# candrewlee14/zgml

Hardware: AMD Instinct MI355X
Metric: decode_tokens_per_sec (higher is better)
Workload: dtype f32; 1 GPU; SmolLM-135M Q4_0 greedy decode, batch 1, 1xMI355X (BASELINE configs[1]); weights=synthetic Q4_0 (int4 + f16 block scale / 32), tied f32 LM head, max_seq=2048, loop=device-resident (inputs in HBM), parallelism=none

## Files before the change

include/zgml_hip.h:

```cpp
#ifndef ZGML_HIP_H
#define ZGML_HIP_H

#include <stddef.h>
#include <stdint.h>

#ifdef __cplusplus
extern "C" {
#endif

#define ZGML_HIP_ABI_VERSION 1

enum {
    ZGML_OP_NONE = 0,
    ZGML_OP_VIEW = 1,
    ZGML_OP_RESHAPE = 2,
    ZGML_OP_TRANSPOSE = 3,
    ZGML_OP_PERMUTE = 4,
    ZGML_OP_AS_STRIDED = 5,
    ZGML_OP_BROADCAST_TO = 6,
    ZGML_OP_ADD = 7,
    ZGML_OP_MUL = 8,
    ZGML_OP_NEG = 9,
    ZGML_OP_ABS = 10,
    ZGML_OP_SGN = 11,
// ... 261 lines not shown


uint64_t zgml_hip_program_plan_text(zgml_hip_ctx* ctx, zgml_hip_program* handle, char* out, uint64_t cap);

enum {
    ZGML_HIP_OPT_FUSION = 1,
    ZGML_HIP_OPT_GRAPH = 2,
    ZGML_HIP_OPT_PROFILE = 3,
    ZGML_HIP_OPT_SKIP_DEAD_UPLOADS = 4,
    ZGML_HIP_OPT_F16_DENSE_WEIGHTS = 5,
    ZGML_HIP_OPT_DENSE_WEIGHT_CACHE = 6,
    ZGML_HIP_OPT_ATTN_SPLIT_MIN_KEYS = 7,
    ZGML_HIP_OPT_FUSE_RESIDENT_WGS = 8,
    ZGML_HIP_OPT_KSPLIT = 9,
    ZGML_HIP_OPT_W8A8 = 10,
    ZGML_HIP_OPT_SMALL_M_MATVEC = 11
};
int zgml_hip_set_option(zgml_hip_ctx* ctx, int option, int64_t value);
void zgml_hip_dense_cache_invalidate(zgml_hip_ctx* ctx, const float* b);
void zgml_hip_dense_cache_stats(zgml_hip_ctx* ctx, uint64_t* hits, uint64_t* misses, uint64_t* bytes);

void* zgml_hip_program_buffer_ptr(zgml_hip_program* handle, uint16_t buf_idx);
int zgml_hip_copy_program_buffer(zgml_hip_ctx* ctx, zgml_hip_program* dst, uint16_t dst_buf, uint64_t dst_offset,
                                 zgml_hip_program* src, uint16_t src_buf, uint64_t src_offset, uint64_t n_elems);
void* zgml_hip_stream(zgml_hip_ctx* ctx);
void zgml_hip_enqueue_program(zgml_hip_ctx* ctx, zgml_hip_program* handle);
void zgml_hip_enqueue_ops(zgml_hip_ctx* ctx, zgml_hip_program* handle, uint64_t first, uint64_t count);
int zgml_hip_program_set_barriers(zgml_hip_ctx* ctx, zgml_hip_program* handle, const uint64_t* op_indices,
                                  uint64_t n);
void zgml_hip_synchronize(zgml_hip_ctx* ctx);
int zgml_hip_stage_inputs(zgml_hip_ctx* ctx, zgml_hip_program* handle, const zgml_program_io* inputs, uint64_t n_inputs);
// ... 122 lines not shown
```

zgml_amd/capi.py:

```python
from __future__ import annotations

import ctypes as C
import os
from pathlib import Path

ABI_VERSION = 1

OP = {
    "none": 0, "view": 1, "reshape": 2, "transpose": 3, "permute": 4, "as_strided": 5,
    "broadcast_to": 6, "add": 7, "mul": 8, "neg": 9, "abs": 10, "sgn": 11, "step": 12,
    "relu": 13, "sqrt": 14, "recip": 15, "exp": 16, "log": 17, "gelu": 18, "sum": 19,
    "max": 20, "repeat": 21,
}
OP_NAME = {v: k for k, v in OP.items()}

DOP_KINDS = [
    "elementwise", "matmul", "qmatmul", "softmax", "layernorm", "rmsnorm", "reduce",
    "repeat", "slice_assign", "rope", "attention", "fused_elementwise",
]
DOP = {name: i for i, name in enumerate(DOP_KINDS)}
DOP.update({"kvq_store": 13, "attention_kvq": 14})


class MatMulGeom(C.Structure):
# ... 187 lines not shown
class ShardPointC(C.Structure):
    _fields_ = [("op_end", C.c_uint64), ("buf_idx", C.c_uint16), ("_pad", C.c_uint16), ("offset", C.c_uint32),
                ("len_per_rank", C.c_uint32)]


class ShardPeerHandleC(C.Structure):
    _fields_ = [("ipc", C.c_ubyte * 64), ("pid", C.c_uint64), ("raw", C.c_uint64), ("bytes", C.c_uint64)]


OPT_FUSION, OPT_GRAPH, OPT_PROFILE, OPT_SKIP_DEAD_UPLOADS, OPT_F16_DENSE_WEIGHTS, OPT_DENSE_WEIGHT_CACHE = 1, 2, 3, 4, 5, 6
OPT_ATTN_SPLIT_MIN_KEYS = 7
OPT_FUSE_RESIDENT_WGS = 8
OPT_KSPLIT = 9
OPT_W8A8 = 10
OPT_SMALL_M_MATVEC = 11

_PKG_DIR = Path(__file__).resolve().parent
HIP_LIB_PATH = _PKG_DIR / "lib" / "libzgml_hip.so"
HOST_LIB_PATH = Path(os.environ["ZGML_HOST_LIB"]) if os.environ.get("ZGML_HOST_LIB") else _PKG_DIR / "lib" / "libzgml_host.so"

_hip_lib = None


def _bind_hip(lib: C.CDLL) -> None:
    vp, u64, u32, i32 = C.c_void_p, C.c_uint64, C.c_uint32, C.c_int
    lib.zgml_hip_create.restype, lib.zgml_hip_create.argtypes = vp, [i32]
    lib.zgml_hip_destroy.restype, lib.zgml_hip_destroy.argtypes = None, [vp]
    lib.zgml_hip_last_error.restype, lib.zgml_hip_last_error.argtypes = C.c_char_p, [vp]
    lib.zgml_hip_clear_error.restype, lib.zgml_hip_clear_error.argtypes = None, [vp]
    lib.zgml_hip_capabilities.restype, lib.zgml_hip_capabilities.argtypes = None, [C.POINTER(CapabilitiesC)]
# ... 120 lines not shown
```

zgml_amd/csrc/kernels.h:

```cpp
#pragma once

#include <hip/hip_runtime.h>
#include <stdint.h>
#include <stdlib.h>

#include "../../include/zgml_hip.h"
#include "switches.h"

namespace zgml {

inline uint32_t device_cus() {
    static const uint32_t n = [] {
        int dev = 0, cus = 0;
        if (hipGetDevice(&dev) != hipSuccess || hipDeviceGetAttribute(&cus, hipDeviceAttributeMultiprocessorCount, dev) != hipSuccess || cus <= 0) cus = 256;
        return (uint32_t)cus;
    }();
    return n;
}

constexpr int kMaxFusedSteps = 8;

struct FusedStepDev {
    uint32_t op;
    uint32_t swapped;
// ... 402 lines not shown
uint32_t qmatmul_max_group();
void launch_qmatmul_group(hipStream_t s, const QWeightDev* w, const QMatmulParams* p, uint32_t n, float* scratch);
bool qmv_prenorm_ok(const QWeightDev& w, uint32_t K, uint64_t total_cols, uint32_t M);
bool qmv_pair_ok(const QWeightDev& w);
bool qmv_can_group(const QWeightDev& a, const QWeightDev& b);
uint32_t qmv_max_prologue_k(const QWeightDev& w);
void launch_qmatvec_fused(hipStream_t s, const QmvLaunch& L);
bool launch_qkv_attention(hipStream_t s, const QmvLaunch& L, const AttnDecodeParams* dev_params, uint32_t n_heads, uint32_t n_kv, uint32_t d_head,
                          const AttnSplit& sp, uint32_t* counters, const uint32_t* idx, uint32_t* seen, uint32_t* timeout,
                          const QmvLaunch* o_proj = nullptr, uint32_t* out_cnt = nullptr, uint32_t* o_seen = nullptr, bool kvq = false);
bool launch_attention_o(hipStream_t s, const AttnDecodeParams* dev_params, uint32_t n_heads, uint32_t d_head, const AttnSplit& sp, const QmvLaunch& o_proj,
                        uint32_t* out_cnt, uint32_t* o_seen, uint32_t* timeout);
int attn_o_blocks_per_cu(uint32_t d_head);
int qkv_attn_kon_census(hipStream_t s, uint32_t d_head, bool kvq, uint32_t grid);
int qkv_attn_kon_blocks_per_cu(uint32_t d_head, bool kvq);
void launch_synth_packed(hipStream_t s, const QWeightDev& w, uint32_t matrix_id);

struct KsVec {
    const float* base = nullptr;
    const float* parts = nullptr;
    uint32_t n_parts = 0;
    float* sum_dst = nullptr;
    float* add_dst = nullptr;
};
struct KsNormIn {
    KsVec x;
    const float* gamma = nullptr;
    float eps = 0.f;
    float* store_mid = nullptr;
    float* store_x = nullptr;
// ... 69 lines not shown
```

zgml_amd/csrc/plan.hip:

```cpp
#include "runtime_internal.h"

namespace {

float* buf_at(zgml_hip_program* p, uint16_t idx, uint64_t off) { return p->bufs[idx] + off; }

template <typename T>
const T* upload_params(zgml_hip_program* p, const std::vector<T>& v) {
    void* d = nullptr;
    if (hipMalloc(&d, v.size() * sizeof(T)) != hipSuccess) {
        p->ctx->fail("plan: parameter array allocation failed");
        return nullptr;
    }
    if (h2d_sync(p->ctx->stream, d, v.data(), v.size() * sizeof(T)) != hipSuccess) p->ctx->fail("plan: parameter array upload failed");
    p->param_blobs.push_back(d);
    return (const T*)d;
}

AttnSplit attn_split_for(zgml_hip_program* p, uint32_t n_heads, uint32_t d_head, uint32_t max_kv, int default_min_keys = 128) {
    const int want = sw().hip_attn_split;
    const int min_keys_env = sw().hip_attn_split_min_keys;
    AttnSplit sp;
    const int64_t min_keys = p->ctx->opt_attn_split_min_keys >= 0 ? p->ctx->opt_attn_split_min_keys : (min_keys_env >= 0 ? min_keys_env : default_min_keys);
    if (min_keys == 0 || want <= 1) return sp;
    sp.min_keys = (uint32_t)std::min<int64_t>(std::max<int64_t>(32, min_keys), 1 << 30);
// ... 899 lines not shown
        bool ok = ga.n_epi == 5 && st[0].op == ZGML_OP_NEG && !st[0].store && st[1].op == ZGML_OP_EXP && st[1].store && st[2].op == ZGML_OP_ADD &&
                  st[2].operand && st[2].operand != ga.dst && st[2].operand != st[1].store && !st[2].store && st[3].op == ZGML_OP_RECIP && !st[3].store &&
                  st[4].op == ZGML_OP_MUL && st[4].operand == ga.dst && st[4].store && up.n_epi == 0;
        ok = ok && ga.w.format == up.w.format && qmv_pair_ok(ga.w) && qmv_pair_ok(up.w) && ga.w.N == up.w.N && ga.w.K == up.w.K && (ga.w.N / 16) % 2 == 0 && ga.w.N == D->K &&
             (G->pro.kind == QMV_PRO_NONE || G->pro.kind == QMV_PRO_PRENORM) && D->n_parts == 1;
        ok = ok && ((D->pro.a == st[4].store && D->pro.b == up.dst) || (D->pro.b == st[4].store && D->pro.a == up.dst));
        ok = ok && (ga.w.format == QW_Q4K || G->pro.kind != QMV_PRO_PRENORM || ga.w.N >= G->K);
        ok = ok && (const char*)up.w.qs == (const char*)ga.w.qs + ga.w.qs_bytes && (const char*)up.w.sc == (const char*)ga.w.sc + ga.w.sc_bytes;
        ok = ok && ((uintptr_t)G->pro.a % 16 == 0) && (G->K % 4 == 0) && (G->pro.kind != QMV_PRO_PRENORM || (uintptr_t)G->pro.xg % 16 == 0);
        if (!ok) continue;
        if (barrier_between_launches(p, i - 1)) continue;
        G->pair_out = D->pro.store_x;
        QmvPrologue plain;
        plain.a = D->pro.store_x;
        D->pro = plain;
    }
}

struct Planner {
    zgml_hip_program* p;
    const std::vector<zgml_device_op>& ops;
    const std::vector<OpAccess>& access;
    const size_t n;
    std::vector<int> owner;
    std::vector<char> in_macro;
    std::vector<Macro> macros;
    struct ProInfo {
        QmvPrologue pro;
        std::vector<uint32_t> absorbed;
        std::vector<uint32_t> consumers;
// ... 772 lines not shown
void build_fused_plan(zgml_hip_program* p) {
    Planner pl(p);
    pl.hoist_constant_repeats();
    pl.prologues();
    pl.matvec_macros();
    pl.decode_attention(false);
    pl.decode_attention(true);
    pl.store_folds();
    pl.row_chains();
    pl.elementwise_chains();
    pl.singletons();
    pl.emit_levels();
    fuse_ksplit(p);
    arm_prenorm(p);
    arm_pair(p);
    fuse_qkv_attention(p);
#ifdef ZGML_TRACE
    fuse_attention_o(p);
#endif
}

}

namespace zgml_rt {

void free_param_blobs(zgml_hip_program* p) {
    for (void* d : p->param_blobs) hipFree(d);
    p->param_blobs.clear();
}

void build_plan(zgml_hip_program* p) {
    {
        hipStreamCaptureStatus st = hipStreamCaptureStatusNone;
        if (hipStreamIsCapturing(p->ctx->stream, &st) == hipSuccess && st != hipStreamCaptureStatusNone) {
            p->ctx->fail("build_plan: the plan has to be rebuilt, but the context's stream is being captured — run one step outside the capture first");
            return;
        }
    }
    hipStreamSynchronize(p->ctx->stream);
    p->plan.clear();
    for (size_t i = 0; i < p->ops.size(); i++) {
        const zgml_device_op& op = p->ops[i];
        if (op.kind == ZGML_DOP_QMATMUL && op.u.qmatmul.M != 1 && op.u.qmatmul.M > p->kon_max_m && op.u.qmatmul.weight_idx < p->qweights.size() &&
            p->qweights[op.u.qmatmul.weight_idx].format == QW_Q4K)
            p->ctx->fail("build_plan: op " + std::to_string(i) + " is an M > " + std::to_string(p->kon_max_m) + " qmatmul over a weight packed for M <= " +
                         std::to_string(p->kon_max_m) + " mat-vecs (K-on-lanes layout)");
    }
    free_param_blobs(p);
    for (void* d : p->fuse_owned) hipFree(d);
    p->fuse_owned.clear();
    p->fuse_epoch = p->ctx->fuse_epoch;
    p->split_buf = nullptr, p->split_cnt = nullptr, p->split_buf_floats = 0, p->split_cnt_words = 0;
    p->split_pos = UINT64_MAX - 1, p->split_input = nullptr, p->qmm_group = nullptr, p->f16_group = nullptr;
    p->plan_batched = p->ctx->opt_fusion && p->batching_safe;
    if (p->plan_batched) {
// ... 23 lines not shown
```

zgml_amd/csrc/qmatvec.hip:

```cpp
#include "qmv_common.h"
#include "attention_decode.h"

#include <hip/hip_fp16.h>
#include <math.h>
#include <stdlib.h>
#include <string.h>

#include <type_traits>
#include <utility>

namespace zgml {

namespace {



struct QMVPartDev {
    const uint4* qs;
    const void* sc;
    float* out;
    uint32_t NB2;
    uint32_t block_begin;
    uint32_t out_rs;
    uint32_t n_epi;
// ... 1496 lines not shown
                         : (fused_kvq ? qkv_attn_kernel<__half, true, 16, true> : qkv_attn_kernel<__half, true, 16, false>);
        else
            ff = prenorm ? (fused_kvq ? qkv_attn_kernel<__half, true, 32, true, 2> : qkv_attn_kernel<__half, true, 32, false, 2>)
                         : (fused_kvq ? qkv_attn_kernel<__half, true, 32, true> : qkv_attn_kernel<__half, true, 32, false>);
        hipLaunchKernelGGL(ff, dim3(total_blocks + extra_blocks), dim3(1024), lds, s, a.parts[0].qs, a.parts[0].sc, a.parts[0].out, head_xa, head_xb, a.in_rs, a.K,
                           head_flags(a, waves, true, rmsnorm, late), nb2_12, a, f);
        return true;
    }
    hipLaunchKernelGGL(fn, grid, dim3(waves * 64), lds, s, a.parts[0].qs, a.parts[0].sc, a.parts[0].out, head_xa, head_xb, a.in_rs, a.K,
                       head_flags(a, waves, contig, rmsnorm, late), nb2_12, a);
    return true;
}

}

uint32_t qmv_max_prologue_k(const QWeightDev& w) { return w.format == QW_Q4K ? UINT32_MAX : kMaxWaves * 64 * 4 * kXRegs; }

void launch_qmatvec_rows(hipStream_t s, const QWeightDev& w, const QMatmulParams& p, bool xvec) {
    QMVArgs a{};
    a.n_parts = 1;
    a.parts[0].qs = (const uint4*)w.qs;
    a.parts[0].sc = w.sc;
    a.parts[0].out = p.dst;
    a.parts[0].NB2 = p.N / 16;
    a.parts[0].block_begin = 0;
    a.parts[0].out_rs = p.dst_rs;
    a.parts[0].n_epi = 0;
    a.pro.kind = QMV_PRO_NONE;
    a.pro.a = p.input;
    a.pro.b = p.input;
// ... 168 lines not shown
```

zgml_amd/csrc/runtime.hip:

```cpp
#include "runtime_internal.h"

namespace zgml_rt {
std::string g_create_error;
}

namespace {


void fill_caps(zgml_capabilities* c) {
    memset(c, 0, sizeof(*c));
    c->compiled_programs = 1;
    c->host_visible_program_memory = 0;
    c->dense_matmul_f32 = 1;
    c->dense_matmul_f16 = 1;
    c->qmatmul = 1;
    c->fused_elementwise = 1;
    c->max_fused_elementwise_steps_has = 1;
    c->max_fused_elementwise_steps = kMaxFusedSteps;
    c->f16_weight_promotion = 1;
    c->dynamic_program_refresh = 1;
    c->prefill_attention = 1;
    c->decode_attention = 1;
    c->quantized_kv = 1;
    c->command_buffer_execution = 1;
// ... 573 lines not shown

int zgml_hip_set_option(zgml_hip_ctx* ctx, int option, int64_t value) {
    if (!ctx) return -1;
    switch (option) {
        case ZGML_HIP_OPT_FUSION: ctx->opt_fusion = value != 0; return 0;
        case ZGML_HIP_OPT_GRAPH: ctx->opt_graph = value != 0; return 0;
        case ZGML_HIP_OPT_PROFILE: ctx->opt_profile = value != 0; return 0;
        case ZGML_HIP_OPT_SKIP_DEAD_UPLOADS: ctx->opt_skip_dead = value != 0; return 0;
        case ZGML_HIP_OPT_F16_DENSE_WEIGHTS: ctx->opt_f16_dense = value != 0; return 0;
        case ZGML_HIP_OPT_ATTN_SPLIT_MIN_KEYS: ctx->opt_attn_split_min_keys = value < 0 ? -1 : value; return 0;
        case ZGML_HIP_OPT_FUSE_RESIDENT_WGS:
            ctx->opt_fuse_resident_wgs = value < 0 ? -1 : value;
            ctx->fuse_epoch++;
            return 0;
        case ZGML_HIP_OPT_KSPLIT: ctx->opt_ksplit = value != 0; return 0;
        case ZGML_HIP_OPT_W8A8: ctx->opt_w8a8 = value != 0; return 0;
        case ZGML_HIP_OPT_SMALL_M_MATVEC:
            ctx->opt_small_m = value <= 0 ? 0 : (value == 1 ? kKonRowsRoutedM : (uint32_t)std::min<int64_t>(value, kKonRowsMaxM));
            return 0;
        case ZGML_HIP_OPT_DENSE_WEIGHT_CACHE:
            ctx->b_cache_cap = value > 0 ? (uint64_t)value : 0;
            if (!ctx->b_cache_cap) ctx->drop_b_cache();
            return 0;
        default: return -1;
    }
}

int zgml_hip_dense_matmul_f32(zgml_hip_ctx* ctx, float* dst, uint64_t dst_len, const float* a, uint64_t a_len,
                              const float* b, uint64_t b_len, const zgml_matmul_geom* g) {
    if (!ctx || !g || !dst || !a || !b) return 0;
// ... 73 lines not shown
    if (hits) *hits = ctx->b_cache_hits;
    if (misses) *misses = ctx->b_cache_misses;
    if (bytes) *bytes = ctx->b_cache_bytes;
}

zgml_hip_program* zgml_hip_compile_program(zgml_hip_ctx* ctx, const zgml_device_program* prog) {
    if (!ctx || !prog) return nullptr;
    if (!program_supported(prog)) {
        ctx->fail("compile_program: program not supported by Capabilities.hip");
        return nullptr;
    }
    hipSetDevice(ctx->device);
    zgml_hip_program* p = new zgml_hip_program();
    p->ctx = ctx;
    p->ksplit = ctx->opt_ksplit;
    own_ops(p, prog->ops, prog->n_ops);
    const size_t nb = prog->n_buffers;
    p->sizes.resize(nb);
    for (size_t i = 0; i < nb; i++) p->sizes[i] = prog->buffer_sizes[i] ? prog->buffer_sizes[i] : 1;

    std::vector<char> live(nb, ctx->opt_skip_dead ? 0 : 1);
    std::vector<uint16_t> ids;
    std::vector<char> qw_live(prog->n_qweights, 0);
    for (const auto& op : p->ops) {
        ids.clear();
        op_buffers(op, ids);
        for (uint16_t id : ids) live[id] = 1;
        if (op.kind == ZGML_DOP_QMATMUL) qw_live[op.u.qmatmul.weight_idx] = 1;
    }

// ... 713 lines not shown
        ctx->fail("copy_program_buffer: range exceeds a buffer");
        return -1;
    }
    unhoist_if_guarded(dst, dst_buf);
    hipSetDevice(ctx->device);
    return CTX_CHECK(ctx, hipMemcpyAsync(dst->bufs[dst_buf] + dst_offset, src->bufs[src_buf] + src_offset, n_elems * sizeof(float),
                                         hipMemcpyDeviceToDevice, ctx->stream))
               ? 0
               : -1;
}

void zgml_hip_enqueue_ops(zgml_hip_ctx* ctx, zgml_hip_program* p, uint64_t first, uint64_t count) {
    if (!ctx || !p) return;
    hipSetDevice(ctx->device);
    if (!p->ksplit_off && !(first == 0 && count >= p->ops.size()))
        p->ksplit_off = true, p->plan_dirty = p->plan_dirty || p->has_deferred;
    ensure_plan(p);
    flush_dyn(p);
    for (auto& L : p->plan) {
        if (L.op_lo >= first && L.op_hi < first + count) {
            L.run(ctx->stream);
        } else if (!(L.op_hi < first || L.op_lo >= first + count)) {
            ctx->fail("enqueue_ops: range cuts through a batched launch; declare it with zgml_hip_program_set_barriers");
            return;
        }
    }
}

int zgml_hip_program_set_barriers(zgml_hip_ctx* ctx, zgml_hip_program* p, const uint64_t* op_indices, uint64_t n) {
    if (!ctx || !p) return -1;
    p->barriers.assign(op_indices, op_indices + n);
// ... 21 lines not shown
```

zgml_amd/csrc/runtime_internal.h:

```cpp
#pragma once
#include <hip/hip_runtime.h>

#include <algorithm>
#include <chrono>
#include <cstdio>
#include <cstdlib>
#include <cstring>
#include <functional>
#include <map>
#include <memory>
#include <string>
#include <vector>

#include "kernels.h"
#include "schedule.h"

using namespace zgml;

namespace zgml_rt {

extern std::string g_create_error;

struct SplitHook {
    const float* out = nullptr;
// ... 47 lines not shown
    bool dyn_row = false;
};

}
using namespace zgml_rt;

struct ShardState;
struct zgml_hip_ctx {
    int device = 0;
    hipStream_t stream = nullptr;
    std::string err;
    bool opt_fusion = true, opt_graph = true, opt_profile = false, opt_skip_dead = true, opt_f16_dense = false;
    bool host_prof = false;
    uint64_t prof_ns[4] = {0, 0, 0, 0}, prof_calls[4] = {0, 0, 0, 0};
    bool opt_ksplit = false;
    bool opt_w8a8 = false;
    uint32_t opt_small_m = 0;
    int64_t opt_attn_split_min_keys = -1;
    int64_t opt_fuse_resident_wgs = -1;
    float *mm_a = nullptr, *mm_b = nullptr, *mm_c = nullptr;
    uint64_t mm_a_cap = 0, mm_b_cap = 0, mm_c_cap = 0;
    struct CachedB {
        float* dev;
        uint64_t span;
    };
    std::map<const float*, CachedB> b_cache;
    uint64_t b_cache_cap = 0, b_cache_bytes = 0, b_cache_hits = 0, b_cache_misses = 0;
    void drop_b_cache() {
        for (auto& kv : b_cache) hipFree(kv.second.dev);
        b_cache.clear();
        b_cache_bytes = 0;
    }
    float* arg_val = nullptr;
    int64_t* arg_idx = nullptr;
    uint32_t* arg_cnt = nullptr;
    int64_t* arg_out = nullptr;
    int64_t* arg_out_host = nullptr;
    uint64_t* smp_keys = nullptr;
    SampleParamsDev* smp_params = nullptr;
    uint32_t* smp_out = nullptr;
    struct ShardState* shard = nullptr;
    uint32_t* handoff_flag = nullptr;
    uint32_t* handoff_flag_dev = nullptr;
    bool fuse_qkv_off = false;
    uint64_t fuse_epoch = 0;
    int n_cu = 0;
    std::map<uint64_t, int> census;
    bool handoff_ok(const char* where) {
        if (!handoff_flag || !*(volatile uint32_t*)handoff_flag) return true;
        const uint32_t cause = *(volatile uint32_t*)handoff_flag;
        *(volatile uint32_t*)handoff_flag = 0;
        if (cause == 2) {
            fail(std::string(where) + ": a peer gather's wait at a gather point timed out (or a peer had already failed the step) — the results of "
                                      "this step are wrong on every rank; all ranks must re-attach (zgml_hip_shard_attach + peer export / import) before stepping again");
            return false;
        }
        fuse_qkv_off = true, fuse_epoch++;
        fail(std::string(where) + ": an in-launch hand-off wait of a fused q/k/v + attention launch timed out — the results of this run are wrong; "
                                  "the fusion is now off for this context (later runs use two launches)");
        return false;
    }

    void fail(const std::string& what) {
        if (err.empty()) err = what;
    }
    bool check(hipError_t e, const char* what) {
        if (e == hipSuccess) return true;
        fail(std::string(what) + ": " + hipGetErrorString(e));
        return false;
// ... 27 lines not shown
    uint64_t split_buf_floats = 0, split_cnt_words = 0;
    bool f16_stream_nt = false;
    std::vector<void*> f16_weights;
    std::vector<void*> owned;
    uint64_t fuse_epoch = 0;
    std::vector<void*> fuse_owned;
    std::vector<char> hoist_op;
    std::vector<char> hoist_guard;
    bool hoist_ok = true;
    bool ksplit = false;
    uint32_t kon_max_m = 1;
    uint32_t n_seqs = 0;
    std::vector<uint32_t> op_seq;
    bool ksplit_off = false;
    bool has_deferred = false;
    float* prenorm_buf = nullptr;
    size_t prenorm_bytes = 0;
    float* scratch = nullptr;
    uint64_t scratch_bytes = 0;
    uint64_t split_pos = UINT64_MAX - 1;
    const float* split_input = nullptr;
    std::shared_ptr<std::vector<std::pair<QWeightDev, QMatmulParams>>> qmm_group;
    std::shared_ptr<std::vector<DenseF16Params>> f16_group;
    uint32_t split_M = 0, split_K = 0, split_in_rs = 0, split_kind = 0;
    uint32_t* dyn_dev = nullptr;
    uint32_t* dyn_host = nullptr;
    bool dyn_dirty = true;
    std::vector<Launch> plan;
    bool plan_dirty = true;
    Schedule sched;
// ... 69 lines not shown
```

Measured before the change: 1672 tokens/s.

## Fuse post-attention O, gate/up and down matvecs into one XCD-local chained launch

```diff
diff --git a/include/zgml_hip.h b/include/zgml_hip.h
--- a/include/zgml_hip.h
+++ b/include/zgml_hip.h
@@ -299,7 +299,8 @@
     ZGML_HIP_OPT_FUSE_RESIDENT_WGS = 8,
     ZGML_HIP_OPT_KSPLIT = 9,
     ZGML_HIP_OPT_W8A8 = 10,
-    ZGML_HIP_OPT_SMALL_M_MATVEC = 11
+    ZGML_HIP_OPT_SMALL_M_MATVEC = 11,
+    ZGML_HIP_OPT_XCD_CHAIN = 12
 };
 int zgml_hip_set_option(zgml_hip_ctx* ctx, int option, int64_t value);
 void zgml_hip_dense_cache_invalidate(zgml_hip_ctx* ctx, const float* b);
diff --git a/zgml_amd/capi.py b/zgml_amd/capi.py
--- a/zgml_amd/capi.py
+++ b/zgml_amd/capi.py
@@ -225,6 +225,7 @@
 OPT_KSPLIT = 9
 OPT_W8A8 = 10
 OPT_SMALL_M_MATVEC = 11
+OPT_XCD_CHAIN = 12
 
 _PKG_DIR = Path(__file__).resolve().parent
 HIP_LIB_PATH = _PKG_DIR / "lib" / "libzgml_hip.so"
diff --git a/zgml_amd/csrc/kernels.h b/zgml_amd/csrc/kernels.h
--- a/zgml_amd/csrc/kernels.h
+++ b/zgml_amd/csrc/kernels.h
@@ -440,6 +440,20 @@
 int attn_o_blocks_per_cu(uint32_t d_head);
 int qkv_attn_kon_census(hipStream_t s, uint32_t d_head, bool kvq, uint32_t grid);
 int qkv_attn_kon_blocks_per_cu(uint32_t d_head, bool kvq);
+uint32_t qmv_waves_of(const QWeightDev& w);
+
+constexpr bool kXcdChainDefault = true;
+struct XcdChainLaunch {
+    QmvLaunch o, gu, down;
+    uint32_t* sync = nullptr;
+    uint32_t* timeout = nullptr;
+    uint32_t P = 32, target_xcc = 0, grid = 256;
+    unsigned long long* trace = nullptr;
+};
+bool xcd_chain_shape_ok(const QmvLaunch& o, const QmvLaunch& gu, const QmvLaunch& down, uint32_t P);
+size_t xcd_chain_sync_words(const QmvLaunch& o, const QmvLaunch& gu);
+bool launch_xcd_chain(hipStream_t s, const XcdChainLaunch& L);
+int xcd_chain_census(hipStream_t s, const QmvLaunch& o, const QmvLaunch& gu, const QmvLaunch& down, uint32_t P, uint32_t target_xcc, uint32_t grid);
 void launch_synth_packed(hipStream_t s, const QWeightDev& w, uint32_t matrix_id);
 
 struct KsVec {
diff --git a/zgml_amd/csrc/plan.hip b/zgml_amd/csrc/plan.hip
--- a/zgml_amd/csrc/plan.hip
+++ b/zgml_amd/csrc/plan.hip
@@ -937,6 +937,72 @@
         QmvPrologue plain;
         plain.a = D->pro.store_x;
         D->pro = plain;
+    }
+}
+
+void fuse_post_attention_chain(zgml_hip_program* p) {
+    p->has_chain = false;
+    zgml_hip_ctx* const ctx = p->ctx;
+    if (!p->xcd_chain || ctx->xcd_chain_off || p->ksplit_off || !p->barriers.empty() || !ctx->handoff_flag_dev || ctx->n_cu < 64) return;
+    const uint32_t P = 32, target_xcc = 0, grid = (uint32_t)ctx->n_cu;
+    auto overlap = [](const float* a, size_t na, const float* b, size_t nb) { return a && b && a < b + nb && b < a + na; };
+    std::map<uint64_t, uint32_t*> sync_of;
+    for (size_t i = 0; i + 2 < p->plan.size(); i++) {
+        const auto O = p->plan[i].qmv_desc, G = p->plan[i + 1].qmv_desc, D = p->plan[i + 2].qmv_desc;
+        if (!O || !G || !D || !xcd_chain_shape_ok(*O, *G, *D, P)) continue;
+        const size_t N0 = O->parts[0].w.N, NG = G->parts[0].w.N, K0 = O->K;
+        {
+            const float* late[2] = {D->parts[0].dst, D->parts[0].epi[0].store};
+            const float* early[5] = {O->pro.a, O->parts[0].epi[0].operand, O->parts[0].epi[0].store, O->next.gamma, G->parts[0].epi[2].operand};
+            const size_t early_n[5] = {K0, N0, N0, N0, NG};
+            bool clash = false;
+            for (const float* l : late)
+                for (int e = 0; e < 5; e++) clash = clash || overlap(l, N0, early[e], early_n[e]);
+            clash = clash || overlap(late[0], N0, late[1], N0) || overlap(G->pair_out, NG, O->next.xg_out, N0 + N0 / 16);
+            if (clash) continue;
+        }
+        const uint64_t key = ((uint64_t)K0 << 40) | ((uint64_t)N0 << 24) | ((uint64_t)NG << 8) | P;
+        auto it = ctx->chain_census.find(key);
+        if (it == ctx->chain_census.end()) {
+            const int r = sw().hip_fuse_census ? xcd_chain_census(ctx->stream, *O, *G, *D, P, target_xcc, grid) : -1;
+            it = ctx->chain_census.emplace(key, r).first;
+            if (r != 1)
+                fprintf(stderr, "[zgml_hip] the post-attention chain launch (%u players on XCC %u) is NOT co-resident on this device (census %d): separate launches instead\n", P,
+                        target_xcc, r);
+        }
+        if (it->second != 1) continue;
+        uint32_t*& sync = sync_of[key];
+        if (!sync) {
+            const size_t words = xcd_chain_sync_words(*O, *G);
+            if (hipMalloc((void**)&sync, words * 4) != hipSuccess) {
+                sync = nullptr;
+                continue;
+            }
+            if (memset_sync(ctx->stream, sync, 0, words * 4) != hipSuccess) {
+                hipFree(sync);
+                sync = nullptr;
+                continue;
+            }
+            p->fuse_owned.push_back(sync);
+        }
+        XcdChainLaunch C;
+        C.o = *O, C.gu = *G, C.down = *D;
+        C.sync = sync, C.timeout = ctx->handoff_flag_dev, C.P = P, C.target_xcc = target_xcc, C.grid = grid;
+#ifdef ZGML_TRACE
+        if (sw().hip_ks_trace && p->ks_traces.size() < 24 && (C.trace = mapped_trace(32)))
+            p->ks_traces.push_back({C.trace, "xcd-chain (ticket | loads issued | o published | seam 1 | gate/up published | seam 2 | end)"});
+#endif
+        const Launch &a = p->plan[i], &b = p->plan[i + 1], &c = p->plan[i + 2];
+        Launch F{ZGML_DOP_QMATMUL, a.n_ops + b.n_ops + c.n_ops, std::min({a.op_lo, b.op_lo, c.op_lo}), std::max({a.op_hi, b.op_hi, c.op_hi}), [C](hipStream_t s) {
+                     if (launch_xcd_chain(s, C)) return;
+                     launch_qmatvec_fused(s, C.o);
+                     launch_qmatvec_fused(s, C.gu);
+                     launch_qmatvec_fused(s, C.down);
+                 }};
+        F.tag = "xcd-chain: O + residual | gate / up pair | down + residual, one launch on one XCD";
+        p->plan[i] = std::move(F);
+        p->plan.erase(p->plan.begin() + (ptrdiff_t)i + 1, p->plan.begin() + (ptrdiff_t)i + 3);
+        p->has_chain = true;
     }
 }
 
@@ -1739,6 +1805,7 @@
     fuse_ksplit(p);
     arm_prenorm(p);
     arm_pair(p);
+    fuse_post_attention_chain(p);
     fuse_qkv_attention(p);
 #ifdef ZGML_TRACE
     fuse_attention_o(p);
@@ -1764,6 +1831,7 @@
     }
     hipStreamSynchronize(p->ctx->stream);
     p->plan.clear();
+    p->has_chain = false;
     for (size_t i = 0; i < p->ops.size(); i++) {
         const zgml_device_op& op = p->ops[i];
         if (op.kind == ZGML_DOP_QMATMUL && op.u.qmatmul.M != 1 && op.u.qmatmul.M > p->kon_max_m && op.u.qmatmul.weight_idx < p->qweights.size() &&
diff --git a/zgml_amd/csrc/qmatvec.hip b/zgml_amd/csrc/qmatvec.hip
--- a/zgml_amd/csrc/qmatvec.hip
+++ b/zgml_amd/csrc/qmatvec.hip
@@ -1534,6 +1534,8 @@
 
 }
 
+uint32_t qmv_waves_of(const QWeightDev& w) { return qmv_waves(w); }
+
 uint32_t qmv_max_prologue_k(const QWeightDev& w) { return w.format == QW_Q4K ? UINT32_MAX : kMaxWaves * 64 * 4 * kXRegs; }
 
 void launch_qmatvec_rows(hipStream_t s, const QWeightDev& w, const QMatmulParams& p, bool xvec) {
diff --git a/zgml_amd/csrc/runtime.hip b/zgml_amd/csrc/runtime.hip
--- a/zgml_amd/csrc/runtime.hip
+++ b/zgml_amd/csrc/runtime.hip
@@ -611,6 +611,7 @@
             ctx->fuse_epoch++;
             return 0;
         case ZGML_HIP_OPT_KSPLIT: ctx->opt_ksplit = value != 0; return 0;
+        case ZGML_HIP_OPT_XCD_CHAIN: ctx->opt_xcd_chain = value != 0; return 0;
         case ZGML_HIP_OPT_W8A8: ctx->opt_w8a8 = value != 0; return 0;
         case ZGML_HIP_OPT_SMALL_M_MATVEC:
             ctx->opt_small_m = value <= 0 ? 0 : (value == 1 ? kKonRowsRoutedM : (uint32_t)std::min<int64_t>(value, kKonRowsMaxM));
@@ -714,6 +715,7 @@
     zgml_hip_program* p = new zgml_hip_program();
     p->ctx = ctx;
     p->ksplit = ctx->opt_ksplit;
+    p->xcd_chain = ctx->opt_xcd_chain;
     own_ops(p, prog->ops, prog->n_ops);
     const size_t nb = prog->n_buffers;
     p->sizes.resize(nb);
@@ -1457,7 +1459,7 @@
     if (!ctx || !p) return;
     hipSetDevice(ctx->device);
     if (!p->ksplit_off && !(first == 0 && count >= p->ops.size()))
-        p->ksplit_off = true, p->plan_dirty = p->plan_dirty || p->has_deferred;
+        p->ksplit_off = true, p->plan_dirty = p->plan_dirty || p->has_deferred || p->has_chain;
     ensure_plan(p);
     flush_dyn(p);
     for (auto& L : p->plan) {
diff --git a/zgml_amd/csrc/runtime_internal.h b/zgml_amd/csrc/runtime_internal.h
--- a/zgml_amd/csrc/runtime_internal.h
+++ b/zgml_amd/csrc/runtime_internal.h
@@ -85,6 +85,7 @@
     bool host_prof = false;
     uint64_t prof_ns[4] = {0, 0, 0, 0}, prof_calls[4] = {0, 0, 0, 0};
     bool opt_ksplit = false;
+    bool opt_xcd_chain = kXcdChainDefault;
     bool opt_w8a8 = false;
     uint32_t opt_small_m = 0;
     int64_t opt_attn_split_min_keys = -1;
@@ -114,8 +115,10 @@
     uint32_t* handoff_flag = nullptr;
     uint32_t* handoff_flag_dev = nullptr;
     bool fuse_qkv_off = false;
+    bool xcd_chain_off = false;
     uint64_t fuse_epoch = 0;
     int n_cu = 0;
+    std::map<uint64_t, int> chain_census;
     std::map<uint64_t, int> census;
     bool handoff_ok(const char* where) {
         if (!handoff_flag || !*(volatile uint32_t*)handoff_flag) return true;
@@ -124,6 +127,12 @@
         if (cause == 2) {
             fail(std::string(where) + ": a peer gather's wait at a gather point timed out (or a peer had already failed the step) — the results of "
                                       "this step are wrong on every rank; all ranks must re-attach (zgml_hip_shard_attach + peer export / import) before stepping again");
+            return false;
+        }
+        if (cause == 3) {
+            xcd_chain_off = true, fuse_epoch++;
+            fail(std::string(where) + ": a seam wait of a post-attention chain launch timed out — the results of this run are wrong; the chain is now off "
+                                      "for this context (later runs use the separate O, gate / up and down launches)");
             return false;
         }
         fuse_qkv_off = true, fuse_epoch++;
@@ -181,6 +190,8 @@
     std::vector<uint32_t> op_seq;
     bool ksplit_off = false;
     bool has_deferred = false;
+    bool xcd_chain = false;
+    bool has_chain = false;
     float* prenorm_buf = nullptr;
     size_t prenorm_bytes = 0;
     float* scratch = nullptr;
diff --git a/zgml_amd/csrc/xcd_chain.hip b/zgml_amd/csrc/xcd_chain.hip
--- /dev/null
+++ b/zgml_amd/csrc/xcd_chain.hip
@@ -0,0 +1,445 @@
+#include "qmv_common.h"
+
+#include <hip/hip_fp16.h>
+#include <math.h>
+
+namespace zgml {
+
+namespace {
+
+constexpr uint32_t kXcWaves = 16;
+constexpr uint32_t kXcMaxLocal = 4;
+constexpr uint32_t kXcLine = 32;
+constexpr uint32_t kXcLds = 96 * 1024;
+constexpr uint32_t kXcTicket = 0, kXcDone = kXcLine, kXcEpoch = 2 * kXcLine, kXcCnt = 3 * kXcLine;
+
+using gu32 = __attribute__((address_space(1))) uint32_t;
+using gf32 = const __attribute__((address_space(1))) float;
+#define XC_RLX __ATOMIC_RELAXED, __HIP_MEMORY_SCOPE_AGENT
+
+struct XcdChainArgs {
+    const uint4* o_qs;
+    const Pair<__half>* o_sc;
+    const float* o_x;
+    float* o_out;
+    const float* o_res;
+    float* h1;
+    const float* gamma2;
+    float* xg;
+    float* ssq;
+    const uint4* g_qs;
+    const Pair<__half>* g_sc;
+    float* gate_out;
+    float* up_out;
+    float* e_store;
+    float* silu_store;
+    const float* ones;
+    float* pair_out;
+    float* store_mid;
+    float* store_x;
+    const uint4* d_qs;
+    const Pair<__half>* d_sc;
+    float* d_out;
+    float* h2;
+    const float* gamma3;
+    float* xg3;
+    float* ssq3;
+    uint32_t* sync;
+    uint32_t* timeout;
+    uint32_t* census;
+    unsigned long long* trace;
+    float eps;
+    uint32_t K0, U0, VW0, NB2_0;
+    uint32_t U1, VW1, NB2_g;
+    uint32_t U2, VW2;
+    uint32_t P, target_xcc, poll_sleep, wait_ticks;
+};
+
+__device__ __forceinline__ uint32_t xcc_id() {
+    uint32_t x;
+    asm volatile("s_getreg_b32 %0, hwreg(HW_REG_XCC_ID)" : "=s"(x));
+    return x & 0xF;
+}
+
+struct XcTask {
+    uint4 wq;
+    Pair<__half> s2;
+    uint32_t vw, loc;
+    bool act;
+};
+
+__device__ __forceinline__ void xc_request(XcTask& k, const uint4* qs, const Pair<__half>* sc, uint32_t t, uint32_t n_tasks, uint32_t VW, uint32_t U, uint32_t NB2,
+                                           uint32_t rank, uint32_t P, uint32_t row, uint32_t i) {
+    k.act = t < n_tasks;
+    const uint32_t tc = k.act ? t : 0;
+    k.loc = (tc >= VW ? 1u : 0u) + (tc >= 2 * VW ? 1u : 0u) + (tc >= 3 * VW ? 1u : 0u), k.vw = tc - k.loc * VW;
+    const uint32_t g = min(rank + P * k.loc, NB2 - 1), ud = min(4 * k.vw + row, U - 1);
+    k.wq = qs[((uint64_t)g * U + ud) * 16 + i];
+    k.s2 = sc[((uint64_t)(g >> 1) * U + ud) * 16 + i];
+}
+__device__ __forceinline__ void xc_xindex(const XcTask& k, uint32_t U, uint32_t K, uint32_t row, uint32_t i, uint32_t& ka, uint32_t& kb) {
+    const uint32_t ud = min(4 * k.vw + row, U - 1);
+    ka = min(ud * 32 + i, K - 1), kb = min(ud * 32 + 16 + i, K - 1);
+}
+__device__ __forceinline__ float xc_compute(const XcTask& k, float xa, float xb, uint32_t U, uint32_t K, uint32_t row, uint32_t i) {
+    const uint32_t ud = 4 * k.vw + row;
+    const bool ok = k.act && ud < U;
+    const uint32_t ka = ud * 32 + i, kb = ka + 16;
+    const float va = ka < K ? xa : 0.f, vb = kb < K ? xb : 0.f;
+    float tA = ok ? (__half2float(k.s2.a) * 16.0f) * va : 0.f;
+    float tB = ok ? (__half2float(k.s2.b) * 16.0f) * vb : 0.f;
+    float acc0 = 0.f, acc1 = 0.f, acc2 = 0.f, acc3 = 0.f;
+    dpp_fence(tA, tB);
+    q4_dword<0>(acc0, acc1, k.wq.x, tA);
+    q4_dword<8>(acc2, acc3, k.wq.y, tA);
+    q4_dword<0>(acc0, acc1, k.wq.z, tB);
+    q4_dword<8>(acc2, acc3, k.wq.w, tB);
+    return rows_sum4((acc0 + acc1) + (acc2 + acc3));
+}
+__device__ __forceinline__ float xc_fold(const float* red, uint32_t VW, uint32_t lane) {
+    const uint32_t r = lane >> 4, col = lane & 15;
+    float part[4];
+#pragma unroll
+    for (uint32_t j = 0; j < 4; j++) part[j] = red[min(r + 4 * j, VW - 1) * 16 + col];
+    float v = 0.f;
+#pragma unroll
+    for (uint32_t j = 0; j < 4; j++) v += r + 4 * j < VW ? part[j] : 0.f;
+    return rows_sum4(v);
+}
+
+__device__ __forceinline__ bool xc_wait(const uint32_t* cnt, uint32_t n, uint32_t target, const XcdChainArgs& a, uint32_t lane) {
+    const unsigned long long t0 = wall_clock64();
+    const uint32_t s0 = min(lane, n - 1), s1 = min(lane + 64, n - 1);
+    for (;;) {
+        const uint32_t c0 = __hip_atomic_load((const gu32*)cnt + (uint64_t)s0 * kXcLine, XC_RLX);
+        const uint32_t c1 = __hip_atomic_load((const gu32*)cnt + (uint64_t)s1 * kXcLine, XC_RLX);
+        if (__all((int32_t)(c0 - target) >= 0 && (int32_t)(c1 - target) >= 0)) return true;
+        if (wall_clock64() - t0 > a.wait_ticks) {
+            if (lane == 0) __hip_atomic_store(a.timeout, 3u, __ATOMIC_RELAXED, __HIP_MEMORY_SCOPE_SYSTEM);
+            return false;
+        }
+        for (uint32_t z = 0; z < a.poll_sleep; z++) __builtin_amdgcn_s_sleep(1);
+    }
+}
+
+__device__ __forceinline__ void xc_leave(const XcdChainArgs& a, uint32_t epoch) {
+    if (threadIdx.x != 0) return;
+    gu32* const sy = (gu32*)a.sync;
+    if (__hip_atomic_fetch_add(sy + kXcDone, 1u, XC_RLX) == gridDim.x - 1) {
+        __hip_atomic_store(sy + kXcTicket, 0u, XC_RLX);
+        __hip_atomic_store(sy + kXcDone, 0u, XC_RLX);
+        __hip_atomic_store(sy + kXcEpoch, epoch + 1, XC_RLX);
+    }
+}
+
+template <int R0, int R1, int R2>
+__global__ void __launch_bounds__(1024) xcd_chain_kernel(XcdChainArgs a) {
+    extern __shared__ float smem[];
+    float* const red = smem;
+    float* const hs = smem + kXcMaxLocal * 2 * 16 * 16;
+    __shared__ uint32_t ctl[2];
+#ifdef ZGML_TRACE
+#define XC_STAMP(i) do { if (a.trace && rank == 0 && threadIdx.x == 0) a.trace[i] = wall_clock64(); } while (0)
+#else
+#define XC_STAMP(i) do { } while (0)
+#endif
+    const uint32_t lane = threadIdx.x & 63, w = __builtin_amdgcn_readfirstlane(threadIdx.x >> 6), row = lane >> 4, i = lane & 15;
+#ifdef ZGML_TRACE
+    const unsigned long long t_start = wall_clock64();
+#endif
+    const uint32_t epoch = __hip_atomic_load((const gu32*)a.sync + kXcEpoch, XC_RLX);
+    if (threadIdx.x == 0) {
+        uint32_t r = 0xFFFFFFFFu;
+        if (xcc_id() == a.target_xcc) {
+            r = __hip_atomic_fetch_add((gu32*)a.sync + kXcTicket, 1u, XC_RLX);
+            if (a.census) __hip_atomic_fetch_add((gu32*)a.census + 2, 1u, XC_RLX);
+        }
+        ctl[0] = r, ctl[1] = 0;
+    }
+    __syncthreads();
+    const uint32_t rank = ctl[0], P = a.P;
+    if (rank >= P) {
+        xc_leave(a, epoch);
+        return;
+    }
+    if (a.census) {
+        if (w == 0) {
+            const unsigned long long t0 = wall_clock64();
+            bool seen = false;
+            while (!(seen = __hip_atomic_load((const gu32*)a.sync + kXcTicket, XC_RLX) >= P) && wall_clock64() - t0 <= a.wait_ticks) __builtin_amdgcn_s_sleep(8);
+            if (lane == 0) __hip_atomic_fetch_add((gu32*)a.census + (seen ? 0 : 1), 1u, XC_RLX);
+        }
+        __syncthreads();
+        xc_leave(a, epoch);
+        return;
+    }
+#ifdef ZGML_TRACE
+    if (a.trace && rank == 0 && threadIdx.x == 0) a.trace[0] = t_start;
+#endif
+    XC_STAMP(1);
+    const uint32_t target = epoch + 1;
+    const uint32_t K0 = a.K0, K1 = a.NB2_0 * 16, K2 = a.NB2_g * 16;
+    const uint32_t nloc0 = a.NB2_0 > rank ? (a.NB2_0 - rank + P - 1) / P : 0, nloc1 = a.NB2_g > rank ? (a.NB2_g - rank + P - 1) / P : 0;
+    if (nloc0 == 0 && nloc1 == 0) {
+        xc_leave(a, epoch);
+        return;
+    }
+    const uint32_t nt0 = nloc0 * a.VW0, nt1 = nloc1 * a.VW1, nt2 = nloc0 * a.VW2;
+    uint32_t* const cnt1 = a.sync + kXcCnt;
+    uint32_t* const cnt2 = cnt1 + (uint64_t)a.NB2_0 * kXcLine;
+
+    XcTask t0[R0], t1a[R1], t1b[R1], t2[R2];
+    float x0a[R0], x0b[R0];
+#pragma unroll
+    for (int r = 0; r < R0; r++) {
+        xc_request(t0[r], a.o_qs, a.o_sc, r * kXcWaves + w, nt0, a.VW0, a.U0, a.NB2_0, rank, P, row, i);
+        uint32_t ka, kb;
+        xc_xindex(t0[r], a.U0, K0, row, i, ka, kb);
+        x0a[r] = a.o_x[ka], x0b[r] = a.o_x[kb];
+    }
+    const uint32_t fcol = lane & 15;
+    const uint32_t fg0 = min(rank + P * min(w, kXcMaxLocal - 1), a.NB2_0 - 1), fg1 = min(rank + P * min(w, kXcMaxLocal - 1), a.NB2_g - 1);
+    const float f_res = a.o_res[fg0 * 16 + fcol], f_gam2 = a.gamma2[fg0 * 16 + fcol];
+    const float f_gam3 = (a.xg3 ? a.gamma3 : a.gamma2)[fg0 * 16 + fcol], f_ones = a.ones[fg1 * 16 + fcol];
+#pragma unroll
+    for (int r = 0; r < R1; r++) {
+        xc_request(t1a[r], a.g_qs, a.g_sc, r * kXcWaves + w, nt1, a.VW1, a.U1, a.NB2_g, rank, P, row, i);
+        t1b[r] = t1a[r];
+        const uint32_t g = min(rank + P * t1a[r].loc, a.NB2_g - 1) + a.NB2_g, ud = min(4 * t1a[r].vw + row, a.U1 - 1);
+        t1b[r].wq = a.g_qs[((uint64_t)g * a.U1 + ud) * 16 + i];
+        t1b[r].s2 = a.g_sc[((uint64_t)(g >> 1) * a.U1 + ud) * 16 + i];
+    }
+#pragma unroll
+    for (int r = 0; r < R2; r++) xc_request(t2[r], a.d_qs, a.d_sc, r * kXcWaves + w, nt2, a.VW2, a.U2, a.NB2_0, rank, P, row, i);
+    XC_STAMP(2);
+    __builtin_amdgcn_sched_barrier(0);
+
+#pragma unroll
+    for (int r = 0; r < R0; r++) {
+        const float v = xc_compute(t0[r], x0a[r], x0b[r], a.U0, K0, row, i);
+        if (t0[r].act && lane < 16) red[((t0[r].loc * 2) * 16 + t0[r].vw) * 16 + lane] = v;
+    }
+    __syncthreads();
+    float f_h = 0.f;
+    if (w < nloc0) {
+        const float v = xc_fold(red + (w * 2) * 256, a.VW0, lane);
+        if (lane < 16) {
+            const uint32_t n = fg0 * 16 + lane;
+            a.o_out[n] = v;
+            f_h = v + f_res;
+            a.h1[n] = f_h;
+            a.xg[n] = f_h * f_gam2;
+            const float sq = row16_sum(f_h * f_h);
+            if (lane == 0) a.ssq[fg0] = sq;
+            hs[w * 16 + lane] = f_h;
+        }
+        asm volatile("s_waitcnt vmcnt(0)" ::: "memory");
+        if (lane == 0) __hip_atomic_store((gu32*)cnt1 + (uint64_t)fg0 * kXcLine, target, XC_RLX);
+    }
+    XC_STAMP(3);
+
+    if (w == 0 && !xc_wait(cnt1, a.NB2_0, target, a, lane)) ctl[1] = 1;
+    __syncthreads();
+    if (ctl[1]) {
+        xc_leave(a, epoch);
+        return;
+    }
+    __builtin_amdgcn_fence(__ATOMIC_ACQUIRE, "wavefront");
+    XC_STAMP(4);
+    float pp[4];
+    {
+        const uint32_t n_ssq = a.NB2_0;
+#pragma unroll
+        for (uint32_t j = 0; j < 4; j++) {
+            const uint32_t q = lane + 64 * j;
+            const float v = __hip_atomic_load((gf32*)a.ssq + min(q, n_ssq - 1), XC_RLX);
+            pp[j] = q < n_ssq ? v : 0.f;
+        }
+    }
+    float x1a[R1], x1b[R1];
+#pragma unroll
+    for (int r = 0; r < R1; r++) {
+        uint32_t ka, kb;
+        xc_xindex(t1a[r], a.U1, K1, row, i, ka, kb);
+        x1a[r] = __hip_atomic_load((gf32*)a.xg + ka, XC_RLX), x1b[r] = __hip_atomic_load((gf32*)a.xg + kb, XC_RLX);
+    }
+    const float inv = 1.0f / sqrtf(rows_sum4(row16_sum((pp[0] + pp[1]) + (pp[2] + pp[3]))) / (float)K1 + a.eps);
+    if (w < nloc0 && lane < 16) {
+        const uint32_t n = fg0 * 16 + lane;
+        const float mid = f_h * inv;
+        if (a.store_mid) a.store_mid[n] = mid;
+        if (a.store_x) a.store_x[n] = mid * f_gam2;
+    }
+
+#pragma unroll
+    for (int r = 0; r < R1; r++) {
+        const float va = xc_compute(t1a[r], x1a[r], x1b[r], a.U1, K1, row, i);
+        const float vb = xc_compute(t1b[r], x1a[r], x1b[r], a.U1, K1, row, i);
+        if (t1a[r].act && lane < 16) {
+            red[((t1a[r].loc * 2) * 16 + t1a[r].vw) * 16 + lane] = va;
+            red[((t1a[r].loc * 2 + 1) * 16 + t1a[r].vw) * 16 + lane] = vb;
+        }
+    }
+    __syncthreads();
+    if (w < nloc1) {
+        float va = xc_fold(red + (w * 2) * 256, a.VW1, lane), vb = xc_fold(red + (w * 2 + 1) * 256, a.VW1, lane);
+        const float f = 1.0f * inv;
+        va *= f, vb *= f;
+        if (lane < 16) {
+            const uint32_t n = fg1 * 16 + lane;
+            a.gate_out[n] = va;
+            a.up_out[n] = vb;
+            const float e = expf(-va);
+            a.e_store[n] = e;
+            const float sl = (1.0f / (e + f_ones)) * va;
+            a.silu_store[n] = sl;
+            a.pair_out[n] = sl * vb;
+        }
+        asm volatile("s_waitcnt vmcnt(0)" ::: "memory");
+        if (lane == 0) __hip_atomic_store((gu32*)cnt2 + (uint64_t)fg1 * kXcLine, target, XC_RLX);
+    }
+    XC_STAMP(5);
+    if (nloc0 == 0) {
+        xc_leave(a, epoch);
+        return;
+    }
+
+    if (w == 0 && !xc_wait(cnt2, a.NB2_g, target, a, lane)) ctl[1] = 1;
+    __syncthreads();
+    if (ctl[1]) {
+        xc_leave(a, epoch);
+        return;
+    }
+    __builtin_amdgcn_fence(__ATOMIC_ACQUIRE, "wavefront");
+    XC_STAMP(6);
+    float x2a[R2], x2b[R2];
+#pragma unroll
+    for (int r = 0; r < R2; r++) {
+        uint32_t ka, kb;
+        xc_xindex(t2[r], a.U2, K2, row, i, ka, kb);
+        x2a[r] = __hip_atomic_load((gf32*)a.pair_out + ka, XC_RLX), x2b[r] = __hip_atomic_load((gf32*)a.pair_out + kb, XC_RLX);
+    }
+
+#pragma unroll
+    for (int r = 0; r < R2; r++) {
+        const float v = xc_compute(t2[r], x2a[r], x2b[r], a.U2, K2, row, i);
+        if (t2[r].act && lane < 16) red[((t2[r].loc * 2) * 16 + t2[r].vw) * 16 + lane] = v;
+    }
+    __syncthreads();
+    if (w < nloc0) {
+        const float v = xc_fold(red + (w * 2) * 256, a.VW2, lane);
+        if (lane < 16) {
+            const uint32_t n = fg0 * 16 + lane;
+            a.d_out[n] = v;
+            const float h = v + hs[w * 16 + lane];
+            a.h2[n] = h;
+            if (a.xg3) {
+                a.xg3[n] = h * f_gam3;
+                const float sq = row16_sum(h * h);
+                if (lane == 0) a.ssq3[fg0] = sq;
+            }
+        }
+    }
+    XC_STAMP(7);
+    xc_leave(a, epoch);
+#undef XC_STAMP
+}
+
+using XcFn = void (*)(XcdChainArgs);
+XcFn xc_pick(uint32_t r0, uint32_t r1, uint32_t r2) {
+    if (r0 == 1 && r1 == 1 && r2 == 1) return xcd_chain_kernel<1, 1, 1>;
+    if (r0 == 1 && r1 == 1 && r2 == 2) return xcd_chain_kernel<1, 1, 2>;
+    if (r0 <= 2 && r1 <= 2 && r2 <= 2) return xcd_chain_kernel<2, 2, 2>;
+    return nullptr;
+}
+
+bool residual_part(const QmvPart& pt) {
+    return pt.n_epi == 1 && pt.epi[0].op == ZGML_OP_ADD && pt.epi[0].operand && pt.epi[0].operand != pt.dst && pt.epi[0].store && pt.epi[0].store != pt.dst;
+}
+bool chain_weight(const QWeightDev& w) { return w.format == QW_Q4 && w.scale_f16 && !w.stream_nt && w.K <= 2048 && w.N % 32 == 0 && w.KC == (w.K + 31) / 32; }
+
+bool xc_args(const QmvLaunch& O, const QmvLaunch& G, const QmvLaunch& D, uint32_t P, XcdChainArgs& a, XcFn& fn) {
+    if (!xcd_chain_shape_ok(O, G, D, P)) return false;
+    const QmvPart &po = O.parts[0], &ga = G.parts[0], &up = G.parts[1], &pd = D.parts[0];
+    a = XcdChainArgs{};
+    a.o_qs = (const uint4*)po.w.qs, a.o_sc = (const Pair<__half>*)po.w.sc, a.o_x = O.pro.a, a.o_out = po.dst, a.o_res = po.epi[0].operand, a.h1 = po.epi[0].store;
+    a.gamma2 = O.next.gamma, a.xg = O.next.xg_out, a.ssq = O.next.ssq_out;
+    a.g_qs = (const uint4*)ga.w.qs, a.g_sc = (const Pair<__half>*)ga.w.sc, a.gate_out = ga.dst, a.up_out = up.dst;
+    a.e_store = ga.epi[1].store, a.silu_store = ga.epi[4].store, a.ones = ga.epi[2].operand, a.pair_out = G.pair_out;
+    a.store_mid = G.pro.store_mid, a.store_x = G.pro.store_x, a.eps = G.pro.eps;
+    a.d_qs = (const uint4*)pd.w.qs, a.d_sc = (const Pair<__half>*)pd.w.sc, a.d_out = pd.dst, a.h2 = pd.epi[0].store;
+    a.gamma3 = D.next.gamma, a.xg3 = D.next.xg_out, a.ssq3 = D.next.ssq_out;
+    a.K0 = po.w.K, a.U0 = po.w.KC, a.VW0 = qmv_waves_of(po.w), a.NB2_0 = po.w.N / 16;
+    a.U1 = ga.w.KC, a.VW1 = qmv_waves_of(ga.w), a.NB2_g = ga.w.N / 16;
+    a.U2 = pd.w.KC, a.VW2 = qmv_waves_of(pd.w);
+    a.P = P;
+    const uint32_t l0 = cdiv(a.NB2_0, P), l1 = cdiv(a.NB2_g, P);
+    fn = xc_pick(cdiv(l0 * a.VW0, kXcWaves), cdiv(l1 * a.VW1, kXcWaves), cdiv(l0 * a.VW2, kXcWaves));
+    return fn != nullptr;
+}
+
+}
+
+bool xcd_chain_shape_ok(const QmvLaunch& O, const QmvLaunch& G, const QmvLaunch& D, uint32_t P) {
+    if (P == 0 || O.n_parts != 1 || G.n_parts != 2 || D.n_parts != 1 || O.trace || G.trace || D.trace) return false;
+    const QmvPart &po = O.parts[0], &ga = G.parts[0], &up = G.parts[1], &pd = D.parts[0];
+    if (!chain_weight(po.w) || !chain_weight(ga.w) || !chain_weight(up.w) || !chain_weight(pd.w)) return false;
+    if (O.pro.kind != QMV_PRO_NONE || !residual_part(po) || !O.next.xg_out || !O.next.ssq_out || !O.next.gamma || O.next.ssq_out != O.next.xg_out + po.w.N) return false;
+    if (G.pro.kind != QMV_PRO_PRENORM || !G.pair_out || G.pro.a != po.epi[0].store || G.pro.b != O.next.gamma || G.pro.xg != O.next.xg_out || G.pro.ssq != O.next.ssq_out ||
+        G.K != po.w.N || G.pro.n_ssq != po.w.N / 16)
+        return false;
+    const QmvEpiStep* st = ga.epi;
+    if (!(ga.n_epi == 5 && st[0].op == ZGML_OP_NEG && !st[0].store && st[1].op == ZGML_OP_EXP && st[1].store && st[2].op == ZGML_OP_ADD && st[2].operand && !st[2].store &&
+          st[3].op == ZGML_OP_RECIP && !st[3].store && st[4].op == ZGML_OP_MUL && st[4].operand == ga.dst && st[4].store && up.n_epi == 0 && sw().qmv_epi_silu))
+        return false;
+    if (ga.w.N != up.w.N || ga.w.K != up.w.K || (const char*)up.w.qs != (const char*)ga.w.qs + ga.w.qs_bytes || (const char*)up.w.sc != (const char*)ga.w.sc + ga.w.sc_bytes) return false;
+    if (D.pro.kind != QMV_PRO_NONE || D.pro.a != G.pair_out || D.K != ga.w.N || !residual_part(pd) || pd.epi[0].operand != po.epi[0].store || pd.w.N != po.w.N) return false;
+    if (D.next.xg_out && (!D.next.ssq_out || !D.next.gamma)) return false;
+    if (po.w.N % 32 || po.w.N > 2048 || ga.w.N > 2048 || !sw().qmv_xdirect) return false;
+    if (ga.w.N < po.w.N) return false;
+    const QWeightDev* ws[3] = {&po.w, &ga.w, &pd.w};
+    for (const QWeightDev* w : ws) {
+        const uint32_t vw = qmv_waves_of(*w);
+        if (vw < 1 || vw > kXcWaves || cdiv(w->KC, vw * 4) != 1) return false;
+    }
+    const uint32_t l0 = cdiv(po.w.N / 16, P), l1 = cdiv(ga.w.N / 16, P);
+    if (l0 > kXcMaxLocal || l1 > kXcMaxLocal) return false;
+    return xc_pick(cdiv(l0 * qmv_waves_of(po.w), kXcWaves), cdiv(l1 * qmv_waves_of(ga.w), kXcWaves), cdiv(l0 * qmv_waves_of(pd.w), kXcWaves)) != nullptr;
+}
+
+size_t xcd_chain_sync_words(const QmvLaunch& O, const QmvLaunch& G) { return (size_t)kXcCnt + ((size_t)O.parts[0].w.N / 16 + G.parts[0].w.N / 16) * kXcLine; }
+
+bool launch_xcd_chain(hipStream_t s, const XcdChainLaunch& L) {
+    XcdChainArgs a;
+    XcFn fn = nullptr;
+    if (!xc_args(L.o, L.gu, L.down, L.P, a, fn)) return false;
+    a.sync = L.sync, a.timeout = L.timeout, a.trace = L.trace;
+    a.target_xcc = L.target_xcc, a.poll_sleep = (uint32_t)sw().hip_handoff_sleep;
+    a.wait_ticks = 2000000u;
+    (void)hipFuncSetAttribute((const void*)fn, hipFuncAttributeMaxDynamicSharedMemorySize, (int)kXcLds);
+    hipLaunchKernelGGL(fn, dim3(L.grid), dim3(kXcWaves * 64), kXcLds, s, a);
+    return true;
+}
+
+int xcd_chain_census(hipStream_t s, const QmvLaunch& O, const QmvLaunch& G, const QmvLaunch& D, uint32_t P, uint32_t target_xcc, uint32_t grid) {
+    XcdChainArgs a;
+    XcFn fn = nullptr;
+    if (!xc_args(O, G, D, P, a, fn)) return -1;
+    const size_t words = xcd_chain_sync_words(O, G) + kXcLine;
+    uint32_t* blk = nullptr;
+    if (hipMalloc((void**)&blk, words * 4) != hipSuccess) return -1;
+    int result = -1;
+    uint32_t host[3] = {0, 1, 0};
+    if (hipMemsetAsync(blk, 0, words * 4, s) == hipSuccess && hipFuncSetAttribute((const void*)fn, hipFuncAttributeMaxDynamicSharedMemorySize, (int)kXcLds) == hipSuccess) {
+        a.sync = blk, a.census = blk + (words - kXcLine), a.timeout = nullptr, a.trace = nullptr;
+        a.target_xcc = target_xcc, a.poll_sleep = 2, a.wait_ticks = 20000u;
+        (void)hipGetLastError();
+        hipLaunchKernelGGL(fn, dim3(grid), dim3(kXcWaves * 64), kXcLds, s, a);
+        if (hipGetLastError() == hipSuccess && hipMemcpyAsync(host, a.census, 12, hipMemcpyDeviceToHost, s) == hipSuccess && hipStreamSynchronize(s) == hipSuccess)
+            result = host[0] == P && host[1] == 0 && host[2] >= P ? 1 : 0;
+    }
+    hipFree(blk);
+    return result;
+}
+
+}
```

New measurement: 1316 tokens/s. 0.787x the previous value.
